# mravanelli/pytorch-kaldi

Measured on AMD Instinct MI355X. Metric: train_frames_per_sec, higher is better.
Workload: dtype bf16

## Files before the change

include/pk_amd.h:

```cpp
#ifndef PK_AMD_H
#define PK_AMD_H

#include <stdint.h>

#ifdef __cplusplus
extern "C" {
#endif

#define PK_PREC_F32 0
#define PK_PREC_BF16 1

#define PK_ACT_LINEAR 0
#define PK_ACT_RELU 1
#define PK_ACT_TANH 2
#define PK_ACT_SIGMOID 3
#define PK_ACT_LEAKY_RELU 4
#define PK_ACT_ELU 5

#define PK_CELL_LIGRU 0
#define PK_CELL_RNN 1
#define PK_CELL_LSTM 2
#define PK_CELL_GRU 3
#define PK_CELL_MINGRU 4

// ... 122 lines not shown
int pk_rec_bwd_bf16(void* stream, int cell, int act, int T, int B, int bidir, int H, const float* U, const float* mask,
                    float mask_scalar, const float* Y, const float* S, const float* dY, float* dP2, uint16_t* dGb,
                    int64_t g_pitch, int prefilled);
int pk_rec_fwd_bf16_ln(void* stream, int cell, int act, int T, int B, int bidir, int H, const float* P,
                       const float* pscale, const float* pshift, const float* U, const float* mask, float mask_scalar,
                       const float* ln_gamma, const float* ln_beta, float ln_eps, float* Y, float* S, float* LNS,
                       uint16_t* Yb, int64_t y_pitch, int prefilled, float* lnwork);
int pk_rec_bwd_bf16_ln(void* stream, int cell, int act, int T, int B, int bidir, int H, const float* U, const float* mask,
                       float mask_scalar, const float* ln_gamma, float ln_eps, const float* Y, const float* S,
                       const float* LNS, const float* dY, float* dP2, uint16_t* dGb, int64_t g_pitch, int prefilled,
                       float* lnwork, float* dln_gamma, float* dln_beta);
void pk_persist2_set_trace(void* dev_buf);
void pk_persist2_set_empty_step(int on);
void pk_persist2_set_mode(int force_safe);
void pk_persist2_set_poll_delay(int units);
void pk_persist2_set_lstm_waves(int waves);
int pk_persist2_get_lstm_waves(void);
void pk_rec_helper_set_mode(int mode);
int pk_rec_helper_get_mode(void);
int pk_rec2p_fwd_bf16(void* stream, int cell, int act, int T, int B, int bidir, int H, const float* P,
                      const float* pscale, const float* pshift, const float* U, const float* mask, float mask_scalar,
                      float* Y, float* S, uint16_t* Yb, uint16_t* Xb, int64_t y_pitch, int prefilled);
int pk_rec2p_bwd_bf16(void* stream, int cell, int act, int T, int B, int bidir, int H, const float* U, const float* mask,
                      float mask_scalar, const float* Y, const float* S, const float* dY, uint16_t* dGb, int64_t g_pitch,
                      int prefilled);
int pk_rec2p_fwd_bf16_ln(void* stream, int cell, int act, int T, int B, int bidir, int H, const float* P,
                         const float* pscale, const float* pshift, const float* U, const float* mask, float mask_scalar,
                         const float* ln_gamma, const float* ln_beta, float ln_eps, float* Y, float* S, float* LNS,
                         uint16_t* Yb, uint16_t* Xb, int64_t y_pitch, int prefilled, float* lnwork);
int pk_rec2p_bwd_bf16_ln(void* stream, int cell, int act, int T, int B, int bidir, int H, const float* U, const float* mask,
                         float mask_scalar, const float* ln_gamma, float ln_eps, const float* Y, const float* S,
                         const float* LNS, const float* dY, uint16_t* dGb, int64_t g_pitch, int prefilled, float* lnwork,
                         float* dln_gamma, float* dln_beta);
unsigned pk_persist2_error_count(void);
void pk_persist2_error_reset(void);

int pk_conv1d_pool_fwd(void* stream, const float* x, const float* w, const float* bias, int B, int Cin, int L,
                       int Cout, int K, int pool, float* y, int32_t* argmax, float* work);
int64_t pk_conv_fwd_work_floats(int Cin, int Cout, int K);
int64_t pk_conv_partial_floats(int B, int Cin, int L, int Cout, int K, int pool);
int pk_conv1d_pool_bwd(void* stream, const float* x, const float* w, const float* dy, const int32_t* argmax, int B,
                       int Cin, int L, int Cout, int K, int pool, float* dw, float* dbias, float* dx,
                       float* partial);

int pk_rmsprop_step(void* stream, float* p, const float* g, float* square_avg, int64_t n, float lr, float alpha,
                    float eps, float weight_decay);
int pk_sgd_step(void* stream, float* p, const float* g, float* momentum_buf, int64_t n, float lr, float momentum,
                float weight_decay, int first_step);
int pk_adam_step(void* stream, float* p, const float* g, float* exp_avg, float* exp_avg_sq, float* max_exp_avg_sq,
                 int64_t n, float lr, float beta1, float beta2, float eps, float weight_decay, int step);
int pk_fused_step(void* stream, int kind, float* p, float* g, float* s0, float* s1, float* s2, int64_t n, float lr, float h0,
                  float h1, float h2, float weight_decay, int step, int zero_grad, const int64_t* segs, int nseg,
                  uint16_t* shadow);

unsigned pk_persist_error_count(void);
void pk_persist_error_reset(void);

int pk_linear_bn_act_bf16_covers(int64_t M, int64_t N, int64_t K);
int pk_linear_bn_act_bf16(void* stream, int M, int N, int K, const uint16_t* xb, int64_t ldx, const uint16_t* wb, int64_t ldw,
                          const float* bias, const float* gamma, const float* beta, float eps, float momentum,
                          float* running_mean, float* running_var, int act, const float* mask, float* z, float* a,
                          float* y, uint16_t* yb, int64_t ldyb, float* mean, float* var);
int pk_gemm_bf16_small_splitk(int M, int N, int K);
int pk_linear_bn_act_bf16_sk(void* stream, int M, int N, int K, const uint16_t* xb, int64_t ldx, const uint16_t* wb,
                             int64_t ldw, const float* bias, const float* gamma, const float* beta, float eps,
                             float momentum, float* running_mean, float* running_var, int act, const float* mask,
                             float* z, float* a, float* y, uint16_t* yb, int64_t ldyb, float* mean, float* var,
                             int splitk, float* ws);
int pk_conv1d_pool_dgrad(void* stream, const float* w, const float* dy, const int32_t* argmax, int B, int Cin, int L, int Cout,
                         int K, int pool, float* dx, float* work);
int pk_conv_bf16_covers(int Cin, int Cout, int K, int pool);
int64_t pk_conv_bf16_work_floats(int B, int Cin, int L, int Cout, int K, int pool, int backward);
int pk_conv1d_pool_fwd_bf16(void* stream, const float* x, const float* w, const float* bias, int B, int Cin, int L, int Cout,
                            int K, int pool, float* y, int32_t* argmax, float* work);
int pk_conv1d_pool_bwd_bf16(void* stream, const float* x, const float* w, const float* dy, const int32_t* argmax, int B,
                            int Cin, int L, int Cout, int K, int pool, float* dw, float* dx, float* work);
int pk_selftest_mfma(void* stream, int* h_bad_count);
int pk_selftest_permlane(void* stream, int* h_bad_count);
int pk_selftest_dpp_row_sum(void* stream, int* h_bad_count);
int pk_selftest_cu_hog(void* stream, int blocks, int usec, float* buf);

typedef struct pk_ark pk_ark;
pk_ark* pk_ark_open(const char* path, int64_t offset);
void pk_ark_close(pk_ark* a);
int pk_ark_next(pk_ark* a, int key_expected, char* key, int keycap, int64_t* rows, int64_t* cols);
int pk_ark_read(pk_ark* a, float* dst);
int pk_ark_skip(pk_ark* a);
int pk_ivec_next(pk_ark* a, char* key, int keycap, int64_t* n);
int pk_ivec_read(pk_ark* a, int32_t* dst);
int pk_context_window(const float* x, int64_t rows, int64_t cols, int left, int right, float* out);
int pk_mean_var_norm(float* x, int64_t rows, int64_t cols);

#ifdef __cplusplus
}
#endif
#endif
```

pytorch-kaldi_amd/_lib.py:

```python
import ctypes
import os
import re
import threading

HERE = os.path.dirname(os.path.abspath(__file__))
LIB_PATH = os.path.join(HERE, "lib", "libpk_amd.so")
HEADER = os.path.join(HERE, "..", "include", "pk_amd.h")

_lock = threading.Lock()
_lib = None

c_void_p, c_int, c_float, c_double, c_int64 = ctypes.c_void_p, ctypes.c_int, ctypes.c_float, ctypes.c_double, ctypes.c_int64
P = c_void_p

SIGNATURES = {
    "pk_version": (c_int, []),
    "pk_last_error": (ctypes.c_char_p, []),
    "pk_num_cu": (c_int, []),
    "pk_gemm": (c_int, [P, c_int, c_int, c_int, c_int, c_float, P, c_int64, c_int64, P, c_int64, c_int64, c_float, P,
                        c_int64, P, c_int, P]),
    "pk_gemm_f32_set_form": (None, [c_int]),
    "pk_gemm_bf16_tile_m": (c_int, [c_int]),
    "pk_gemm_bf16_auto_splitk": (c_int, [c_int, c_int, c_int]),
    "pk_gemm_bf16_set_tile": (None, [c_int]),
# ... 46 lines not shown
    "pk_conv1d_pool_fwd_bf16": (c_int, [P, P, P, P, c_int, c_int, c_int, c_int, c_int, c_int, P, P, P]),
    "pk_conv1d_pool_bwd_bf16": (c_int, [P, P, P, P, P, c_int, c_int, c_int, c_int, c_int, c_int, P, P, P]),
    "pk_bn_act_bwd_small_covers": (c_int, [c_int64, c_int64]),
    "pk_bn_act_bwd_small": (c_int, [P, P, P, P, c_int, P, P, P, c_float, P, c_int64, c_int64, P, c_int64, P, P, P, P, P, P, P]),
    "pk_rec_work_floats": (c_int64, [c_int, c_int, c_int, c_int, c_int]),
    "pk_rec_ln_saved_floats": (c_int64, [c_int, c_int, c_int, c_int]),
    "pk_rec_ln_work_floats": (c_int64, [c_int, c_int, c_int, c_int]),
    "pk_rec_fwd": (c_int, [P, c_int, c_int, c_int, c_int, c_int, c_int, c_int, c_int, P, P, P, P, P, c_float, P, P, P,
                           P, P, P]),
    "pk_rec_bwd": (c_int, [P, c_int, c_int, c_int, c_int, c_int, c_int, c_int, c_int, P, P, c_float, P, P, P, P, P, P,
                           P, P, P, P]),
    "pk_rec_self_fill": (c_int, [c_int]),
    "pk_rec_plan_cus": (c_int, [c_int, c_int]),
    "pk_gemm_bf16_auto_splitk_cus": (c_int, [c_int, c_int, c_int, c_int]),
    "pk_rec_fwd_bf16": (c_int, [P, c_int, c_int, c_int, c_int, c_int, c_int, P, P, P, P, P, c_float, P, P, P, c_int64, c_int]),
    "pk_rec_bwd_bf16": (c_int, [P, c_int, c_int, c_int, c_int, c_int, c_int, P, P, c_float, P, P, P, P, P, c_int64, c_int]),
    "pk_rec2p_fwd_bf16_ln": (c_int, [P, c_int, c_int, c_int, c_int, c_int, c_int, P, P, P, P, P, c_float, P, P, c_float, P, P, P,
                                     P, P, c_int64, c_int, P]),
    "pk_rec2p_bwd_bf16_ln": (c_int, [P, c_int, c_int, c_int, c_int, c_int, c_int, P, P, c_float, P, c_float, P, P, P, P, P,
                                     c_int64, c_int, P, P, P]),
    "pk_rec_fwd_bf16_ln": (c_int, [P, c_int, c_int, c_int, c_int, c_int, c_int, P, P, P, P, P, c_float, P, P, c_float, P, P, P,
                                   P, c_int64, c_int, P]),
    "pk_rec_bwd_bf16_ln": (c_int, [P, c_int, c_int, c_int, c_int, c_int, c_int, P, P, c_float, P, c_float, P, P, P, P, P, P,
                                   c_int64, c_int, P, P, P]),
    "pk_rec2p_fwd_bf16": (c_int, [P, c_int, c_int, c_int, c_int, c_int, c_int, P, P, P, P, P, c_float, P, P, P, P, c_int64, c_int]),
    "pk_rec2p_bwd_bf16": (c_int, [P, c_int, c_int, c_int, c_int, c_int, c_int, P, P, c_float, P, P, P, P, c_int64, c_int]),
    "pk_persist2_set_trace": (None, [P]),
    "pk_persist2_set_empty_step": (None, [c_int]),
    "pk_persist2_set_mode": (None, [c_int]),
    "pk_persist2_set_poll_delay": (None, [c_int]),
    "pk_persist2_set_lstm_waves": (None, [c_int]),
    "pk_rec_helper_set_mode": (None, [c_int]),
    "pk_rec_helper_get_mode": (c_int, []),
    "pk_persist2_get_lstm_waves": (c_int, []),
    "pk_persist2_error_count": (ctypes.c_uint, []),
    "pk_persist2_error_reset": (None, []),
    "pk_conv1d_pool_fwd": (c_int, [P, P, P, P, c_int, c_int, c_int, c_int, c_int, c_int, P, P, P]),
    "pk_conv_fwd_work_floats": (c_int64, [c_int, c_int, c_int]),
    "pk_conv_partial_floats": (c_int64, [c_int, c_int, c_int, c_int, c_int, c_int]),
    "pk_conv1d_pool_bwd": (c_int, [P, P, P, P, P, c_int, c_int, c_int, c_int, c_int, c_int, P, P, P, P]),
    "pk_ark_open": (P, [ctypes.c_char_p, c_int64]),
    "pk_ark_close": (None, [P]),
    "pk_ark_next": (c_int, [P, c_int, ctypes.c_char_p, c_int, ctypes.POINTER(c_int64), ctypes.POINTER(c_int64)]),
    "pk_ark_read": (c_int, [P, P]),
    "pk_ark_skip": (c_int, [P]),
    "pk_ivec_next": (c_int, [P, ctypes.c_char_p, c_int, ctypes.POINTER(c_int64)]),
    "pk_ivec_read": (c_int, [P, P]),
    "pk_context_window": (c_int, [P, c_int64, c_int64, c_int, c_int, P]),
    "pk_mean_var_norm": (c_int, [P, c_int64, c_int64]),
    "pk_rmsprop_step": (c_int, [P, P, P, P, c_int64, c_float, c_float, c_float, c_float]),
    "pk_sgd_step": (c_int, [P, P, P, P, c_int64, c_float, c_float, c_float, c_int]),
    "pk_adam_step": (c_int, [P, P, P, P, P, P, c_int64, c_float, c_float, c_float, c_float, c_float, c_int]),
    "pk_fused_step": (c_int, [P, c_int, P, P, P, P, P, c_int64, c_float, c_float, c_float, c_float, c_float, c_int, c_int, P, c_int, P]),
    "pk_persist_error_count": (ctypes.c_uint, []),
    "pk_persist_error_reset": (None, []),
    "pk_linear_bn_act_bf16_covers": (c_int, [c_int64, c_int64, c_int64]),
    "pk_linear_bn_act_bf16": (c_int, [P, c_int, c_int, c_int, P, c_int64, P, c_int64, P, P, P, c_float, c_float, P, P, c_int, P,
                                      P, P, P, P, c_int64, P, P]),
    "pk_gemm_bf16_small_splitk": (c_int, [c_int, c_int, c_int]),
    "pk_linear_bn_act_bf16_sk": (c_int, [P, c_int, c_int, c_int, P, c_int64, P, c_int64, P, P, P, c_float, c_float, P, P, c_int, P,
                                         P, P, P, P, c_int64, P, P, c_int, P]),
    "pk_selftest_mfma": (c_int, [P, ctypes.POINTER(c_int)]),
    "pk_selftest_permlane": (c_int, [P, ctypes.POINTER(c_int)]),
    "pk_selftest_dpp_row_sum": (c_int, [P, ctypes.POINTER(c_int)]),
    "pk_selftest_cu_hog": (c_int, [P, c_int, c_int, P]),
}


def declared_symbols():
    with open(HEADER) as f:
        text = re.sub(r"/\*.*?\*/", "", f.read(), flags=re.S)
    return sorted(set(re.findall(r"\b(pk_[a-z0-9_]+)\s*\(", text)))


class PkError(RuntimeError):
    pass


def _map_torch_hip_runtime():
    import torch

    hip = os.path.join(os.path.dirname(torch.__file__), "lib", "libamdhip64.so")
    if os.path.exists(hip):
        ctypes.CDLL(hip, mode=ctypes.RTLD_GLOBAL)
    return hip


def hip_runtimes_mapped():
    try:
        with open("/proc/self/maps") as f:
            return {line.split()[-1] for line in f if "libamdhip64" in line}
    except OSError:
        return set()


def load():
    global _lib
    if _lib is not None:
        return _lib
    with _lock:
        if _lib is not None:
            return _lib
        if not os.path.exists(LIB_PATH):
            raise PkError(
                "libpk_amd.so is not built (%s). Run `python -c 'import __graft_entry__ as g; g.build()'`; "
                "this engine has no CPU fallback." % LIB_PATH)
# ... 169 lines not shown
```

pytorch-kaldi_amd/csrc/pk_optim.hip:

```cpp
#include "pk_common.h"

namespace {

__global__ void rmsprop_kernel(float* __restrict__ p, const float* __restrict__ g, float* __restrict__ sq, long n, float lr,
                               float alpha, float eps, float wd) {
    for (long i = blockIdx.x * (long)blockDim.x + threadIdx.x; i < n; i += (long)gridDim.x * blockDim.x) {
        float gv = g[i];
        const float pv = p[i];
        if (wd != 0.f) gv += wd * pv;
        const float s = alpha * sq[i] + (1.f - alpha) * gv * gv;
        sq[i] = s;
        p[i] = pv - lr * gv / (sqrtf(s) + eps);
    }
}

__global__ void sgd_kernel(float* __restrict__ p, const float* __restrict__ g, float* __restrict__ buf, long n, float lr,
                           float momentum, float wd, int first) {
    for (long i = blockIdx.x * (long)blockDim.x + threadIdx.x; i < n; i += (long)gridDim.x * blockDim.x) {
        float gv = g[i];
        const float pv = p[i];
        if (wd != 0.f) gv += wd * pv;
        if (momentum != 0.f) {
            const float b = first ? gv : momentum * buf[i] + gv;
            buf[i] = b;
            gv = b;
        }
        p[i] = pv - lr * gv;
    }
}

__global__ void adam_kernel(float* __restrict__ p, const float* __restrict__ g, float* __restrict__ m, float* __restrict__ v,
                            float* __restrict__ vmax, long n, float lr, float beta1, float beta2, float eps, float wd,
                            float bc1, float bc2s) {
    for (long i = blockIdx.x * (long)blockDim.x + threadIdx.x; i < n; i += (long)gridDim.x * blockDim.x) {
        float gv = g[i];
        const float pv = p[i];
        if (wd != 0.f) gv += wd * pv;
        const float mv = beta1 * m[i] + (1.f - beta1) * gv;
        float vv = beta2 * v[i] + (1.f - beta2) * gv * gv;
        m[i] = mv;
        v[i] = vv;
        if (vmax != nullptr) {
            vv = fmaxf(vmax[i], vv);
            vmax[i] = vv;
        }
        const float denom = sqrtf(vv) / bc2s + eps;
        p[i] = pv - (lr / bc1) * (mv / denom);
    }
}

template <int KIND>
__global__ void fused_step_kernel(float* __restrict__ p, float* __restrict__ g, float* __restrict__ s0, float* __restrict__ s1,
                                  float* __restrict__ s2, long n, float lr, float h0, float h1, float h2, float wd, float bc1,
                                  float bc2s, int first, int zero_grad, const long* __restrict__ segs, int nseg,
                                  unsigned short* __restrict__ shadow) {
    for (long i = 4 * (blockIdx.x * (long)blockDim.x + threadIdx.x); i < n; i += 4 * (long)gridDim.x * blockDim.x) {
        f32x4 gv = *reinterpret_cast<const f32x4*>(g + i);
        f32x4 pv = *reinterpret_cast<const f32x4*>(p + i);
        if (wd != 0.f) {
#pragma unroll
            for (int e = 0; e < 4; ++e) gv[e] += wd * pv[e];
        }
        if (KIND == 0) {
            f32x4 sq = *reinterpret_cast<const f32x4*>(s0 + i);
#pragma unroll
            for (int e = 0; e < 4; ++e) {
                sq[e] = h0 * sq[e] + (1.f - h0) * gv[e] * gv[e];
                pv[e] = pv[e] - lr * gv[e] / (sqrtf(sq[e]) + h1);
            }
            *reinterpret_cast<f32x4*>(s0 + i) = sq;
        } else if (KIND == 1) {
            if (h0 != 0.f) {
                f32x4 b = *reinterpret_cast<const f32x4*>(s0 + i);
#pragma unroll
                for (int e = 0; e < 4; ++e) {
                    b[e] = first ? gv[e] : h0 * b[e] + gv[e];
                    gv[e] = b[e];
                }
                *reinterpret_cast<f32x4*>(s0 + i) = b;
            }
#pragma unroll
            for (int e = 0; e < 4; ++e) pv[e] = pv[e] - lr * gv[e];
        } else {
            f32x4 m = *reinterpret_cast<const f32x4*>(s0 + i), v = *reinterpret_cast<const f32x4*>(s1 + i);
            f32x4 vm = v;
#pragma unroll
            for (int e = 0; e < 4; ++e) {
                m[e] = h0 * m[e] + (1.f - h0) * gv[e];
                v[e] = h1 * v[e] + (1.f - h1) * gv[e] * gv[e];
                vm[e] = v[e];
            }
            *reinterpret_cast<f32x4*>(s0 + i) = m;
            *reinterpret_cast<f32x4*>(s1 + i) = v;
            if (s2 != nullptr) {
                const f32x4 old = *reinterpret_cast<const f32x4*>(s2 + i);
#pragma unroll
                for (int e = 0; e < 4; ++e) vm[e] = fmaxf(old[e], v[e]);
                *reinterpret_cast<f32x4*>(s2 + i) = vm;
            }
#pragma unroll
            for (int e = 0; e < 4; ++e) pv[e] = pv[e] - (lr / bc1) * (m[e] / (sqrtf(vm[e]) / bc2s + h2));
        }
        *reinterpret_cast<f32x4*>(p + i) = pv;
        if (zero_grad) *reinterpret_cast<f32x4*>(g + i) = f32x4{0.f, 0.f, 0.f, 0.f};
        if (nseg > 0) {
            int lo = 0, hi = nseg;
            while (hi - lo > 1) {
                const int mid = (lo + hi) >> 1;
                if (segs[5 * mid] <= i) lo = mid;
                else hi = mid;
            }
            const long off = segs[5 * lo], rows = segs[5 * lo + 1], cols = segs[5 * lo + 2], pitch = segs[5 * lo + 3], soff = segs[5 * lo + 4];
            const long rel = i - off;
            if (rel >= 0 && rel < rows * cols) {
                const long row = rel / cols, col = rel - row * cols;
                uint2 pk;
                pk.x = pk_pack_bf2(pv[0], pv[1]);
                pk.y = pk_pack_bf2(pv[2], pv[3]);
                *reinterpret_cast<uint2*>(shadow + soff + row * pitch + col) = pk;
            }
        }
    }
}

inline int blocks_for(long n) {
    long b = (n + 255) / 256;
    if (b > 4096) b = 4096;
    if (b < 1) b = 1;
    return (int)b;
}

}

extern "C" int pk_rmsprop_step(void* stream, float* p, const float* g, float* square_avg, int64_t n, float lr, float alpha,
                               float eps, float weight_decay) {
    if (n == 0) return 0;
    hipLaunchKernelGGL(rmsprop_kernel, dim3(blocks_for(n)), dim3(256), 0, pk_stream(stream), p, g, square_avg, (long)n, lr,
                       alpha, eps, weight_decay);
    PK_LAUNCH_CHECK();
    return 0;
}

extern "C" int pk_sgd_step(void* stream, float* p, const float* g, float* momentum_buf, int64_t n, float lr,
                           float momentum, float weight_decay, int first_step) {
    if (n == 0) return 0;
    PK_REQUIRE(momentum == 0.f || momentum_buf != nullptr, "pk_sgd_step: momentum needs a buffer");
    hipLaunchKernelGGL(sgd_kernel, dim3(blocks_for(n)), dim3(256), 0, pk_stream(stream), p, g, momentum_buf, (long)n, lr,
                       momentum, weight_decay, first_step);
    PK_LAUNCH_CHECK();
    return 0;
}

extern "C" int pk_adam_step(void* stream, float* p, const float* g, float* exp_avg, float* exp_avg_sq, float* max_exp_avg_sq,
                            int64_t n, float lr, float beta1, float beta2, float eps, float weight_decay, int step) {
    if (n == 0) return 0;
    PK_REQUIRE(step >= 1 && exp_avg != nullptr && exp_avg_sq != nullptr, "pk_adam_step: step counts from 1 and needs both moments");
    const float bc1 = 1.f - powf(beta1, (float)step);
    const float bc2s = sqrtf(1.f - powf(beta2, (float)step));
    hipLaunchKernelGGL(adam_kernel, dim3(blocks_for(n)), dim3(256), 0, pk_stream(stream), p, g, exp_avg, exp_avg_sq,
                       max_exp_avg_sq, (long)n, lr, beta1, beta2, eps, weight_decay, bc1, bc2s);
    PK_LAUNCH_CHECK();
    return 0;
}

extern "C" int pk_fused_step(void* stream, int kind, float* p, float* g, float* s0, float* s1, float* s2, int64_t n, float lr,
                             float h0, float h1, float h2, float weight_decay, int step, int zero_grad, const int64_t* segs,
                             int nseg, uint16_t* shadow) {
    if (n == 0) return 0;
    PK_REQUIRE(kind >= 0 && kind <= 2 && step >= 1, "pk_fused_step: kind 0..2, step counts from 1");
    PK_REQUIRE((n & 3) == 0 && (((uintptr_t)p | (uintptr_t)g | (uintptr_t)s0 | (uintptr_t)s1 | (uintptr_t)s2) & 15) == 0,
               "pk_fused_step: n and the buffers must be multiples of 4 elements / 16-byte aligned");
    PK_REQUIRE(kind != 0 || s0 != nullptr, "pk_fused_step: RMSprop needs its square average");
    PK_REQUIRE(kind != 1 || h0 == 0.f || s0 != nullptr, "pk_fused_step: momentum needs a buffer");
    PK_REQUIRE(kind != 2 || (s0 != nullptr && s1 != nullptr), "pk_fused_step: Adam needs both moments");
    PK_REQUIRE(nseg == 0 || (segs != nullptr && shadow != nullptr && ((uintptr_t)shadow & 7) == 0), "pk_fused_step: null segment table / copy");
    const float bc1 = kind == 2 ? 1.f - powf(h0, (float)step) : 1.f;
    const float bc2s = kind == 2 ? sqrtf(1.f - powf(h1, (float)step)) : 1.f;
    const dim3 grid(blocks_for(n / 4)), block(256);
    hipStream_t st = pk_stream(stream);
    const long* sg = reinterpret_cast<const long*>(segs);
    if (kind == 0) hipLaunchKernelGGL(fused_step_kernel<0>, grid, block, 0, st, p, g, s0, s1, s2, (long)n, lr, h0, h1, h2, weight_decay, bc1, bc2s, 0, zero_grad, sg, nseg, (unsigned short*)shadow);
    else if (kind == 1) hipLaunchKernelGGL(fused_step_kernel<1>, grid, block, 0, st, p, g, s0, s1, s2, (long)n, lr, h0, h1, h2, weight_decay, bc1, bc2s, step == 1 ? 1 : 0, zero_grad, sg, nseg, (unsigned short*)shadow);
    else hipLaunchKernelGGL(fused_step_kernel<2>, grid, block, 0, st, p, g, s0, s1, s2, (long)n, lr, h0, h1, h2, weight_decay, bc1, bc2s, 0, zero_grad, sg, nseg, (unsigned short*)shadow);
    PK_LAUNCH_CHECK();
    return 0;
}
```

pytorch-kaldi_amd/functional.py:

```python
import ctypes
import os
import weakref

import torch

from . import _lib

PREC = {"fp32": 0, "bf16": 1}
ACT = {"linear": 0, "relu": 1, "tanh": 2, "sigmoid": 3, "leaky_relu": 4, "elu": 5}
CELL = {"liGRU": 0, "RNN": 1, "LSTM": 2, "GRU": 3, "minimalGRU": 4}
REC_STEPWISE, REC_PERSISTENT = 0, 1


class _Settings:

    def __init__(self):
        self.precision = os.environ.get("PK_PRECISION", "fp32")
        self.rec_algo = os.environ.get("PK_REC_ALGO", "auto")
        self.mask_rng = os.environ.get("PK_MASK_RNG", "device")
        assert self.mask_rng in ("reference", "reference_host", "device"), self.mask_rng
        self.wgrad_side = _lib.experiment("wgrad_side", "1") != "0"
        self.self_fill = _lib.experiment("rec_self_fill", "1") != "0"
        self.side_late = _lib.experiment("side_late", "1") != "0"
        self.side_cus = _lib.experiment("side_cus", "0") != "0"
# ... 233 lines not shown


def _rows2d(x):
    if x.dim() != 2:
        x = x.reshape(-1, x.shape[-1])
    if x.stride(1) != 1 or (x.shape[0] > 1 and x.stride(0) < x.shape[1]):
        x = x.contiguous()
    return x


def _new(*shape, like):
    return torch.empty(*shape, device=like.device, dtype=torch.float32)


def _splitk(out_tiles, K):
    if K < 4096:
        return 1
    slots = int(_lib.experiment("f32_splitk_slots", "1024"))
    s = max(1, slots // max(1, out_tiles))
    return int(min(16, s, max(1, K // 1024)))


def _small_m_splitk(M, N, K):
    if M > 256 or K < 512 or _lib.experiment("f32_small_splitk", "1") == "0":
        return 1
    return int(max(1, min(16, 512 // max(1, _tiles(M, N)), K // 64)))


def gemm(M, N, K, A, a_rs, a_cs, B, b_rs, b_cs, C, ldc, alpha=1.0, beta=0.0, bias=None, splitk=1, prec=None):
    lib = _lib.load()
    ws = None
    if splitk == 1 and a_cs == 1 and (prec or settings.precision) == "fp32":
        splitk = _small_m_splitk(M, N, K)
    if splitk > 1:
        ws = torch.empty(splitk * M * N, device=C.device, dtype=torch.float32)
    rc = lib.pk_gemm(_stream(), PREC[prec or settings.precision], M, N, K, alpha, _p(A), a_rs, a_cs, _p(B), b_rs, b_cs,
                     beta, _p(C), ldc, _p(bias), splitk, _p(ws))
    _lib.check(rc, "pk_gemm")
    return C


def _tiles(M, N):
    return ((M + 127) // 128) * ((N + 127) // 128)


def _tiles_bf(M, N):
    return (M, N)


def _up(n, m):
    return (n + m - 1) // m * m


def weight_bf16(w):
    sh = getattr(w, "_pk_shadow", None)
    if sh is not None:
        view, version, alive, flat_version = sh
        if alive() is not None:
            owner = getattr(w, "_pk_owner", None)
            owner = owner() if owner is not None else None
            fv = owner.flat._version if owner is not None else flat_version
            if w._version == version and fv == flat_version:
                return view
            cvt_bf16(w.detach(), out=view)
            w._pk_shadow = (view, w._version, alive, fv)
            return view
    owner = getattr(w, "_pk_owner", None)
    owner = owner() if owner is not None else None
    if owner is not None and w.is_contiguous():
        owner.want_shadow(w)
    return cvt_bf16(w.contiguous())


def cvt_bf16(x2, nseg=1, seglen=None, segpad=None, out=None):
    lib = _lib.load()
    rows, cols = x2.shape
    if seglen is None:
        nseg, seglen = 1, cols
    if segpad is None:
        segpad = _up(seglen, 8)
    assert nseg * seglen == cols and x2.stride(1) == 1
    pitch = _up(nseg * segpad, 64)
    if out is None:
        out = torch.empty(rows, pitch, device=x2.device, dtype=torch.bfloat16)
    assert tuple(out.shape) == (rows, pitch) and out.dtype == torch.bfloat16 and out.is_contiguous()
    _lib.check(lib.pk_cvt_bf16(_stream(), _p(x2), x2.stride(0), rows, nseg, seglen, segpad, _p(out), pitch),
               "pk_cvt_bf16")
    return out


_SMALL_SPLITK = _lib.experiment("small_splitk", "1") != "0"


def gemm_bf16(M, N, K, A, lda, a_kc, B, ldb, b_kc, C, ldc, alpha=1.0, beta=0.0, bias=None, splitk=1):
    lib = _lib.load()
    ws = None
    if splitk == 1 and a_kc and M <= 128 and _SMALL_SPLITK:
        splitk = int(lib.pk_gemm_bf16_small_splitk(M, N, K))
    if splitk > 1:
        ws = torch.empty(splitk * M * N, device=C.device, dtype=torch.float32)

    def ptr(t):
        if isinstance(t, tuple):
            return ctypes.c_void_p(t[0].data_ptr() + 2 * t[1])
        return ctypes.c_void_p(t.data_ptr())

    rc = lib.pk_gemm_bf16(_stream(), M, N, K, alpha, ptr(A), lda, int(a_kc), ptr(B), ldb, int(b_kc), beta, _p(C), ldc,
                          _p(bias), splitk, _p(ws))
    _lib.check(rc, "pk_gemm_bf16")
    return C


def gemm_bf16_bn_stats(M, N, K, A, lda, a_kc, B, ldb, b_kc, C, ldc, bias=None, gates=None):
    lib = _lib.load()

    def done(mean, var):
        return (mean, var) if gates is None else (mean, var) + tuple(bn_finalize_gates(mean, var, *gates))

    if _lib.experiment("gemm_stats", "1") == "0":
        gemm_bf16(M, N, K, A, lda, a_kc, B, ldb, b_kc, C, ldc, bias=bias)
        return done(*bn_stats(C if ldc == N else C.as_strided((M, N), (ldc, 1))))
    stats = torch.empty(int(lib.pk_gemm_bf16_stats_floats(M, N)), device=C.device, dtype=torch.float32)
    rb = ctypes.c_int(0)
    rc = lib.pk_gemm_bf16_stats(_stream(), M, N, K, 1.0, _p(A), lda, int(a_kc), _p(B), ldb, int(b_kc), _p(C), ldc, _p(bias),
# ... 1265 lines not shown
    if cell not in ("liGRU", "RNN", "LSTM", "GRU", "minimalGRU") or H > 576 or use_ln:
        return False
    return training or not use_bn or not torch.is_grad_enabled()


class _Prefill:
    stream = None

    def __init__(self):
        self.done = 0

    def start(self, *bufs):
        if not settings.wgrad_side:
            return
        main = torch.cuda.current_stream()
        if _Prefill.stream is None:
            _Prefill.stream = torch.cuda.Stream()
        st = _Prefill.stream
        st.wait_stream(main)
        with torch.cuda.stream(st):
            for b in bufs:
                if b is not None:
                    b.view(torch.int16).fill_(-1)
        for b in bufs:
            if b is not None:
                b.record_stream(st)
        self.done = 1

    def wait(self):
        if self.done:
            torch.cuda.current_stream().wait_stream(_Prefill.stream)


class RecLayerPerfFn(torch.autograd.Function):

    @staticmethod
    def forward(ctx, x, xb_in, Wcat, bcat, Ucat, gamma, beta, running_mean, running_var, mask, cfg, edge=None):
        ctx.set_materialize_grads(False)
        _need_gpu(x, Wcat, bcat, Ucat, gamma, beta, mask)
        lib = _lib.load()
        cell, act, H, bidir, use_bn, training, eps, momentum, mask_scalar, xseg = cfg[:10]
        ctx.wparams, ctx.uparams = (cfg[10], cfg[11]) if len(cfg) > 10 else (None, None)
        ctx.side_w, ctx.side_u = (bool(cfg[12]), bool(cfg[13])) if len(cfg) > 13 else (False, False)
        ctx.affine = cfg[15] if len(cfg) > 15 else None
        T, B, D = x.shape
        G = lib.pk_rec_num_gates(CELL[cell])
        NS = lib.pk_rec_num_saved(CELL[cell])
        ndir = 2 if bidir else 1
        TB, GH = T * B, G * H
        Wcat = Wcat.contiguous()
        Ucat = Ucat.contiguous()
        if xb_in is None:
            xseg = None
            xb, Wb, K = cvt_bf16(_rows2d(x)), cvt_bf16(Wcat), D
        else:
            nseg, seglen, segpad = xseg
            assert nseg * seglen == D and xb_in.shape[0] == TB
            xb, Wb, K = xb_in, cvt_bf16(Wcat, nseg, seglen, segpad), nseg * segpad
            assert Wb.shape[1] == xb.shape[1]
        Hp = _up(H, 8)
        Yb = torch.empty(TB, _up(ndir * Hp, 64), device=x.device, dtype=torch.bfloat16)
        two_phase = cell in ("GRU", "minimalGRU")
        self_fill = settings.self_fill and lib.pk_rec_self_fill(CELL[cell]) == 1
        dGb = None
        if any(ctx.needs_input_grad) and not self_fill:
            dGb = torch.empty(ndir * TB, _up(G * Hp, 64), device=x.device, dtype=torch.bfloat16)
        Xb = torch.empty_like(Yb) if two_phase else None
        fill = _Prefill()
        if not self_fill:
            fill.start(Yb, Xb, dGb)
        P = _new(TB, GH, like=Wcat)
        mean = var = None
        bn_bufs = cfg[14] if len(cfg) > 14 else None
        pscale = pshift = None
        if use_bn and training and bn_bufs is not None:
            mean, var, pscale, pshift = gemm_bf16_bn_stats(TB, GH, K, xb, xb.shape[1], 1, Wb, Wb.shape[1], 1, P, GH, gates=(
                gamma, beta, eps, H, bn_bufs[0], bn_bufs[1], bn_bufs[2], momentum, ndir * TB))
        elif use_bn and training:
            mean, var = gemm_bf16_bn_stats(TB, GH, K, xb, xb.shape[1], 1, Wb, Wb.shape[1], 1, P, GH)
        else:
            gemm_bf16(TB, GH, K, xb, xb.shape[1], 1, Wb, Wb.shape[1], 1, P, GH)
        if use_bn:
            if pscale is not None:
                pass
            elif training:
                pscale, pshift = bn_finalize(mean, var, gamma, beta, eps, running_mean, running_var, momentum, ndir * TB)
            else:
                mean, var = running_mean, running_var
                pscale, pshift = bn_finalize(mean, var, gamma, beta, eps)
        else:
            pscale = torch.ones(GH, device=x.device)
            pshift = bcat.contiguous() if bcat is not None else torch.zeros(GH, device=x.device)
        infer = not any(ctx.needs_input_grad) and _Kinks.queue is None and _lib.experiment("fwd_nosave", "1") != "0"
        keep_y = bool(cfg[16]) if len(cfg) > 16 else True
        Y = _new(T, B, ndir * H, like=Wcat)
        S = None if infer else _new(ndir, TB, NS * H, like=Wcat)
        Yarg = Y if (keep_y or not infer) else None
        _lib.raise_if_persist_failed()
        fill.wait()
        if two_phase:
            rc = lib.pk_rec2p_fwd_bf16(_stream(), CELL[cell], ACT[act], T, B, int(bidir), H, _p(P), _p(pscale),
                                       _p(pshift), _p(Ucat), _p(mask), float(mask_scalar), _p(Yarg), _p(S), _p(Yb), _p(Xb),
                                       Yb.shape[1], 2 if self_fill else fill.done)
            _lib.check(rc, "pk_rec2p_fwd_bf16")
        else:
            rc = lib.pk_rec_fwd_bf16(_stream(), CELL[cell], ACT[act], T, B, int(bidir), H, _p(P), _p(pscale), _p(pshift),
                                     _p(Ucat), _p(mask), float(mask_scalar), _p(Yarg), _p(S), _p(Yb), Yb.shape[1],
                                     2 if self_fill else fill.done)
            _lib.check(rc, "pk_rec_fwd_bf16")
        if S is not None:
            _force_kinks(S, cell, T, B, ndir, H)
# ... 56 lines not shown
        elif not side_u:
            do_dU()
        dPb = torch.empty(TB, _up(GH, 64), device=dY.device, dtype=torch.bfloat16)
        part = _new(int(lib.pk_bn_partial_floats(TB, GH)), like=dY)
        sum_g = _new(GH, like=dY)
        sum_gx = _new(GH, like=dY) if use_bn else None
        g1 = ctypes.c_void_p(dGb.data_ptr() + 2 * TB * Gp) if bidir else None
        acc_g = acc_b = None
        if use_bn and ctx.affine is not None:
            acc_g = adjacent_view([q.grad for q in ctx.affine[0]])
            acc_b = adjacent_view([q.grad for q in ctx.affine[1]])
            if acc_g is None or acc_b is None:
                raise _lib.PkError("perf-mode recurrent layer: the BatchNorm gradients left the flat buffer between forward "
                                   "and backward (optim.FlatParams.zero_grad() re-aliases them)")
        rc = lib.pk_bn_bwd_bf16(_stream(), _p(dGb), g1, Gp, G, H, _p(P), GH, TB, _p(mean) if use_bn else None,
                                _p(var) if use_bn else None, eps, _p(gamma) if use_bn else None, float(TB), _p(part),
                                _p(sum_g), _p(sum_gx), _p(dPb), dPb.shape[1], _p(acc_b), _p(acc_g))
        _lib.check(rc, "pk_bn_bwd_bf16")
        dgamma = dbeta = dbias = None
        if use_bn and acc_g is None:
            dgamma, dbeta = sum_gx, sum_g
        elif not use_bn and ctx.has_bias:
            dbias = sum_g
        Kx = D if xseg is None else xseg[0] * xseg[2]
        dWp = _new(GH, Kx, like=dY)
        dW = None

        def do_dW():
            nonlocal dW
            gview = adjacent_view([q.grad for q in ctx.wparams]) if side_w else None
            sk = _splitk_bf(_tiles_bf(GH, Kx), TB)
            if gview is not None and xseg is None:
                gemm_bf16(GH, Kx, TB, dPb, dPb.shape[1], 0, xb, xb.shape[1], 0, gview, Kx, beta=1.0, splitk=sk)
                return
            gemm_bf16(GH, Kx, TB, dPb, dPb.shape[1], 0, xb, xb.shape[1], 0, dWp, Kx, splitk=sk)
            if gview is not None:
                nseg, seglen, segpad = xseg
                with torch.no_grad():
                    for s_ in range(nseg):
                        gview[:, s_ * seglen:(s_ + 1) * seglen].add_(dWp[:, s_ * segpad:s_ * segpad + seglen])
                return
            if xseg is None:
                dW = dWp
            else:
                nseg, seglen, segpad = xseg
                dW = torch.cat([dWp[:, s_ * segpad:s_ * segpad + seglen] for s_ in range(nseg)], 1)
            if side_w:
                _accumulate_rows(ctx.wparams, [dW[g * H:(g + 1) * H] for g in range(G)])

        if side_w and not late:
            side_launch(do_dW, (dPb, xb, dWp), ctx.wparams)
        dx = None
        if ctx.needs_input_grad[0]:
            Wb2 = Wb if xseg is None else cvt_bf16(Wcat)
            dx = _new(TB, D, like=dY)
            gemm_bf16(TB, D, GH, dPb, dPb.shape[1], 1, Wb2, Wb2.shape[1], 0, dx, D)
            dx = dx.view(T, B, D)
        if late:
            free = 0
            if settings.side_cus:
                held = int(lib.pk_rec_plan_cus(ndir * B, H))
                free = max(int(lib.pk_num_cu()) - held, 0) if held > 0 else 0
            if side_u:
                side_launch(_sized_for(free, do_dU), (Y, S, Yb, dGb, Xb, dU), ctx.uparams)
            if side_w:
                side_launch(_sized_for(free, do_dW), (dPb, xb, dWp), ctx.wparams)
        if not side_w:
            do_dW()
        return dx, None, (None if side_w else dW), dbias, (None if side_u else dU), dgamma, dbeta, None, None, None, None, None


CONV_BF16_DEFAULT = "1"


def conv_bf16_mode():
    return os.environ.get("PK_CONV_BF16", CONV_BF16_DEFAULT)


class ConvPoolFn(torch.autograd.Function):
    @staticmethod
    def forward(ctx, x, w, bias, pool):
        _need_gpu(x, w, bias)
        lib = _lib.load()
        x = x.contiguous()
        w = w.contiguous()
        B, Cin, L = x.shape
        Cout, _, K = w.shape
        Lp = (L - K + 1) // pool
        y = _new(B, Cout, Lp, like=x)
        arg = torch.empty(B, Cout, Lp, device=x.device, dtype=torch.int32)
        mode = conv_bf16_mode()
        ctx.conv_bf = (bf16_mode() and mode in ("1", "2") and (Cin >= 8 or mode == "2")
                       and lib.pk_conv_bf16_covers(Cin, Cout, K, pool) == 1)
        if ctx.conv_bf:
            work = _new(int(lib.pk_conv_bf16_work_floats(B, Cin, L, Cout, K, pool, 0)), like=x)
            _lib.check(lib.pk_conv1d_pool_fwd_bf16(_stream(), _p(x), _p(w), _p(bias), B, Cin, L, Cout, K, pool, _p(y),
                                                   ctypes.c_void_p(arg.data_ptr()), _p(work)), "pk_conv1d_pool_fwd_bf16")
        else:
            work = _new(int(lib.pk_conv_fwd_work_floats(Cin, Cout, K)), like=x)
            _lib.check(lib.pk_conv1d_pool_fwd(_stream(), _p(x), _p(w), _p(bias), B, Cin, L, Cout, K, pool, _p(y),
                                              ctypes.c_void_p(arg.data_ptr()), _p(work)), "pk_conv1d_pool_fwd")
        if _Decisions.pool is not None:
            fpool, off = _Decisions.pool.pop(0)
            assert fpool == pool and tuple(off.shape) == (B, Cout, Lp), (fpool, pool, tuple(off.shape), (B, Cout, Lp))
            forced = (torch.arange(Lp, device=x.device, dtype=torch.int32) * pool)[None, None, :] + off.to(x.device).to(torch.int32)
            _Decisions.report.append(("pool", int((forced != arg).sum()), arg.numel()))
            arg = forced.contiguous()
# ... 38 lines not shown
```

pytorch-kaldi_amd/optim.py:

```python
import ctypes
import os
import weakref

import torch

from . import _lib


def _stream():
    return ctypes.c_void_p(torch.cuda.current_stream().cuda_stream)


class FlatParams:
    def __init__(self, module, align=64):
        self.module = module
        self.params = [p for p in module.parameters()]
        dev = self.params[0].device
        unused = {id(p) for p in module.pk_unused_parameters()} if hasattr(module, "pk_unused_parameters") else set()
        self.unused = [id(p) in unused for p in self.params]
        index = {id(p): i for i, p in enumerate(self.params)}
        units, placed = [], set()
        if hasattr(module, "pk_flat_groups") and _lib.experiment("flat_groups", "1") != "0":
            for grp in module.pk_flat_groups():
                ids = [index[id(q)] for q in grp if id(q) in index and id(q) not in unused and index[id(q)] not in placed]
                if ids:
                    units.append(ids)
                    placed.update(ids)
        for i in range(len(self.params)):
            if not self.unused[i] and i not in placed:
                units.append([i])
        self.offsets = [0] * len(self.params)
        off = 0
        for ids in units:
            off = (off + align - 1) // align * align
            for i in ids:
                self.offsets[i] = off
                off += self.params[i].numel()
        off = (off + align - 1) // align * align
        self.n_active = off
        for i, p in enumerate(self.params):
            if self.unused[i]:
                self.offsets[i] = off
                off += (p.numel() + align - 1) // align * align
        self.numel = off
        self.flat = torch.zeros(off, device=dev, dtype=torch.float32)
        self.grad = torch.zeros(off, device=dev, dtype=torch.float32)
        with torch.no_grad():
            for p, o in zip(self.params, self.offsets):
                n = p.numel()
                self.flat[o:o + n].copy_(p.detach().reshape(-1))
                p.data = self.flat[o:o + n].view(p.shape)
                p.grad = self.grad[o:o + n].view(p.shape)
                p._pk_flat = True
                p._pk_owner = weakref.ref(self)
        self._index = {id(p): i for i, p in enumerate(self.params)}
        self._clean = False
        self._shadow_req = set()
        self._shadow_have = ()
        self.shadow = self.shadow_segs = None

    def want_shadow(self, p):
        i = self._index.get(id(p))
        if (i is not None and not self.unused[i] and p.dim() == 2 and p.shape[1] % 4 == 0 and self.offsets[i] % 4 == 0
                and p.is_cuda):
            self._shadow_req.add(i)

    def invalidate_shadows(self):
        for p in self.params:
            sh = getattr(p, "_pk_shadow", None)
            if sh is not None:
                p._pk_shadow = (sh[0], -1, sh[2], -1)

    def build_shadows(self):
        from . import functional as F_
        want = tuple(sorted(self._shadow_req, key=lambda i: self.offsets[i]))
        if want == self._shadow_have:
            return
        rows = []
        soff = 0
        for i in want:
            p = self.params[i]
            pitch = (p.shape[1] + 63) // 64 * 64
            rows.append((self.offsets[i], p.shape[0], p.shape[1], pitch, soff))
            soff += p.shape[0] * pitch
        self.shadow = torch.zeros(max(soff, 8), device=self.flat.device, dtype=torch.bfloat16)
        self.shadow_segs = torch.tensor(rows, dtype=torch.int64, device=self.flat.device).reshape(-1, 5)
        self._shadow_have = want
        for i, (_o, r, c, pitch, so) in zip(want, rows):
            p = self.params[i]
            view = self.shadow[so:so + r * pitch].view(r, pitch)
            F_.cvt_bf16(p.detach(), out=view)
            p._pk_shadow = (view, p._version, weakref.ref(self.shadow), self.flat._version)

    def zero_grad(self):
        from .functional import join_side
        join_side()
        if self._clean:
            self._clean = False
        else:
            self.grad.zero_()
        for p, o in zip(self.params, self.offsets):
            if p.grad is None or p.grad.data_ptr() != self.grad.data_ptr() + 4 * o:
                p.grad = self.grad[o:o + p.numel()].view(p.shape)


def _flat_mark_dirty(self):
    self._clean = False


FlatParams.mark_dirty = _flat_mark_dirty


class FusedOptimizer:

    _STATE_KEYS = {"rmsprop": ("square_avg",), "sgd": ("momentum_buffer",),
                   "adam": ("exp_avg", "exp_avg_sq", "max_exp_avg_sq")}

    def __init__(self, flat, kind, lr, alpha=0.99, eps=1e-8, momentum=0.0, weight_decay=0.0, centered=False,
                 dampening=0.0, nesterov=False, betas=(0.9, 0.999), amsgrad=False):
        if kind not in ("rmsprop", "sgd", "adam"):
            raise _lib.PkError("fused optimizer covers rmsprop, sgd and adam (got %s)" % kind)
        if kind == "rmsprop" and (momentum != 0.0 or centered):
            raise _lib.PkError("fused RMSprop is the momentum-free, non-centred form every shipped recipe uses")
        if kind == "sgd" and (dampening != 0.0 or nesterov):
            raise _lib.PkError("fused SGD does not implement dampening / nesterov")
        self.flat, self.kind, self.lr = flat, kind, lr
        self.alpha, self.eps, self.momentum, self.weight_decay = alpha, eps, momentum, weight_decay
        self.betas, self.amsgrad = tuple(betas), bool(amsgrad)
        z = lambda: torch.zeros_like(flat.flat)
        self.bufs = {}
        if kind == "rmsprop":
            self.bufs["square_avg"] = z()
        elif kind == "sgd" and momentum != 0.0:
            self.bufs["momentum_buffer"] = z()
        elif kind == "adam":
            self.bufs["exp_avg"], self.bufs["exp_avg_sq"] = z(), z()
            if self.amsgrad:
                self.bufs["max_exp_avg_sq"] = z()
        self.steps = 0
        self.param_groups = [{"lr": lr}]
        self.zero_in_step = False

    @property
    def state(self):
        return next(iter(self.bufs.values()), None)

    def zero_grad(self):
        self.flat.zero_grad()

    def step(self):
        if not self.flat.flat.is_cuda:
            raise _lib.PkError("fused optimizer step runs on the GPU only (no CPU fallback)")
        from .functional import join_side
        join_side()
        lib = _lib.load()
        lr = float(self.param_groups[0]["lr"])
        f = self.flat
        ptr = lambda k: self.bufs[k].data_ptr() if k in self.bufs else None
        if f.n_active % 4 == 0 and _lib.experiment("fused_step", "1") != "0":
            if f._shadow_req and not torch.cuda.is_current_stream_capturing():
                f.build_shadows()
            nseg = len(f._shadow_have)
            zero = bool(self.zero_in_step) and _lib.experiment("opt_zero_in_step", "1") != "0"
            kind = {"rmsprop": 0, "sgd": 1, "adam": 2}[self.kind]
            h = {"rmsprop": (self.alpha, self.eps, 0.0), "sgd": (self.momentum, 0.0, 0.0),
                 "adam": (self.betas[0], self.betas[1], self.eps)}[self.kind]
            s0 = ptr("square_avg") if kind == 0 else ptr("momentum_buffer") if kind == 1 else ptr("exp_avg")
            rc = lib.pk_fused_step(_stream(), kind, f.flat.data_ptr(), f.grad.data_ptr(), s0, ptr("exp_avg_sq"),
                                   ptr("max_exp_avg_sq"), f.n_active, lr, h[0], h[1], h[2], self.weight_decay, self.steps + 1,
                                   int(zero), f.shadow_segs.data_ptr() if nseg else None, nseg,
                                   f.shadow.data_ptr() if nseg else None)
            _lib.check(rc, "fused optimizer step")
            f._clean = zero
            self.steps += 1
            return
        if self.kind == "rmsprop":
            rc = lib.pk_rmsprop_step(_stream(), f.flat.data_ptr(), f.grad.data_ptr(), ptr("square_avg"), f.n_active, lr,
                                     self.alpha, self.eps, self.weight_decay)
        elif self.kind == "sgd":
            rc = lib.pk_sgd_step(_stream(), f.flat.data_ptr(), f.grad.data_ptr(), ptr("momentum_buffer"), f.n_active, lr,
                                 self.momentum, self.weight_decay, int(self.steps == 0))
        else:
            rc = lib.pk_adam_step(_stream(), f.flat.data_ptr(), f.grad.data_ptr(), ptr("exp_avg"), ptr("exp_avg_sq"),
                                  ptr("max_exp_avg_sq"), f.n_active, lr, self.betas[0], self.betas[1], self.eps,
                                  self.weight_decay, self.steps + 1)
        _lib.check(rc, "fused optimizer step")
        self.steps += 1

    def _torch_twin(self):
        import torch.optim as optim
        ps = self.flat.params
        lr = float(self.param_groups[0]["lr"])
        if self.kind == "rmsprop":
            return optim.RMSprop(ps, lr=lr, alpha=self.alpha, eps=self.eps, weight_decay=self.weight_decay)
        if self.kind == "sgd":
            return optim.SGD(ps, lr=lr, momentum=self.momentum, weight_decay=self.weight_decay)
        return optim.Adam(ps, lr=lr, betas=self.betas, eps=self.eps, weight_decay=self.weight_decay, amsgrad=self.amsgrad)

    def state_dict(self):
        sd = self._torch_twin().state_dict()
        state = {}
        if self.steps > 0:
            for i, (p, o) in enumerate(zip(self.flat.params, self.flat.offsets)):
                if self.flat.unused[i]:
                    continue
                ent = {k: b[o:o + p.numel()].view(p.shape).clone() for k, b in self.bufs.items()}
                if self.kind != "sgd":
                    ent["step"] = torch.tensor(float(self.steps))
                if ent:
                    state[i] = ent
        sd["state"] = state
        return sd

    def load_state_dict(self, sd):
        groups = sd["param_groups"]
        if len(groups) != 1 or len(groups[0]["params"]) != len(self.flat.params):
            raise _lib.PkError("optimizer state does not match this architecture's parameter list")
        g = groups[0]
        self.param_groups[0]["lr"] = g["lr"]
        self.weight_decay = float(g.get("weight_decay", self.weight_decay))
        if self.kind == "rmsprop":
# ... 48 lines not shown
```

Measured before the change: 3.816 million.

## Cache bf16 shadows of concatenated recurrent weights, refreshed inside fused optimizer step

Extends the optimizer's bf16 shadow mechanism to concatenated recurrent weight matrices, including segmented or padded layouts. The fused step kernel now writes these bf16 copies directly, using an 8-wide segment descriptor that carries segment length and padding. The recurrent layer forward and backward passes then reuse the cached copy instead of converting the fp32 weight to bf16 on every call. This adds a multi-segment lookup with scattered stores to the optimizer kernel, and shadow rebuilds now depend on a simple size signature, which could miss changes in the request set.

```diff
diff --git a/include/pk_amd.h b/include/pk_amd.h
--- a/include/pk_amd.h
+++ b/include/pk_amd.h
@@ -198,6 +198,9 @@
 int pk_fused_step(void* stream, int kind, float* p, float* g, float* s0, float* s1, float* s2, int64_t n, float lr, float h0,
                   float h1, float h2, float weight_decay, int step, int zero_grad, const int64_t* segs, int nseg,
                   uint16_t* shadow);
+int pk_fused_step_seg(void* stream, int kind, float* p, float* g, float* s0, float* s1, float* s2, int64_t n, float lr,
+                      float h0, float h1, float h2, float weight_decay, int step, int zero_grad, const int64_t* segs,
+                      int nseg, uint16_t* shadow);
 
 unsigned pk_persist_error_count(void);
 void pk_persist_error_reset(void);
diff --git a/pytorch-kaldi_amd/_lib.py b/pytorch-kaldi_amd/_lib.py
--- a/pytorch-kaldi_amd/_lib.py
+++ b/pytorch-kaldi_amd/_lib.py
@@ -122,6 +122,7 @@
     "pk_sgd_step": (c_int, [P, P, P, P, c_int64, c_float, c_float, c_float, c_int]),
     "pk_adam_step": (c_int, [P, P, P, P, P, P, c_int64, c_float, c_float, c_float, c_float, c_float, c_int]),
     "pk_fused_step": (c_int, [P, c_int, P, P, P, P, P, c_int64, c_float, c_float, c_float, c_float, c_float, c_int, c_int, P, c_int, P]),
+    "pk_fused_step_seg": (c_int, [P, c_int, P, P, P, P, P, c_int64, c_float, c_float, c_float, c_float, c_float, c_int, c_int, P, c_int, P]),
     "pk_persist_error_count": (ctypes.c_uint, []),
     "pk_persist_error_reset": (None, []),
     "pk_linear_bn_act_bf16_covers": (c_int, [c_int64, c_int64, c_int64]),
diff --git a/pytorch-kaldi_amd/csrc/pk_optim.hip b/pytorch-kaldi_amd/csrc/pk_optim.hip
--- a/pytorch-kaldi_amd/csrc/pk_optim.hip
+++ b/pytorch-kaldi_amd/csrc/pk_optim.hip
@@ -53,7 +53,7 @@
 __global__ void fused_step_kernel(float* __restrict__ p, float* __restrict__ g, float* __restrict__ s0, float* __restrict__ s1,
                                   float* __restrict__ s2, long n, float lr, float h0, float h1, float h2, float wd, float bc1,
                                   float bc2s, int first, int zero_grad, const long* __restrict__ segs, int nseg,
-                                  unsigned short* __restrict__ shadow) {
+                                  int segw, unsigned short* __restrict__ shadow) {
     for (long i = 4 * (blockIdx.x * (long)blockDim.x + threadIdx.x); i < n; i += 4 * (long)gridDim.x * blockDim.x) {
         f32x4 gv = *reinterpret_cast<const f32x4*>(g + i);
         f32x4 pv = *reinterpret_cast<const f32x4*>(p + i);
@@ -107,17 +107,28 @@
             int lo = 0, hi = nseg;
             while (hi - lo > 1) {
                 const int mid = (lo + hi) >> 1;
-                if (segs[5 * mid] <= i) lo = mid;
+                if (segs[segw * mid] <= i) lo = mid;
                 else hi = mid;
             }
-            const long off = segs[5 * lo], rows = segs[5 * lo + 1], cols = segs[5 * lo + 2], pitch = segs[5 * lo + 3], soff = segs[5 * lo + 4];
-            const long rel = i - off;
-            if (rel >= 0 && rel < rows * cols) {
+            const long off = segs[segw * lo];
+            for (; lo >= 0 && segs[segw * lo] == off; --lo) {
+                const long* sg = segs + segw * lo;
+                const long rows = sg[1], cols = sg[2], pitch = sg[3], soff = sg[4];
+                const long rel = i - off;
+                if (rel < 0 || rel >= rows * cols) continue;
                 const long row = rel / cols, col = rel - row * cols;
-                uint2 pk;
-                pk.x = pk_pack_bf2(pv[0], pv[1]);
-                pk.y = pk_pack_bf2(pv[2], pv[3]);
-                *reinterpret_cast<uint2*>(shadow + soff + row * pitch + col) = pk;
+                const long seglen = segw > 5 ? sg[5] : cols, segpad = segw > 5 ? sg[6] : cols;
+                unsigned short* dst = shadow + soff + row * pitch;
+                if (seglen == cols) {
+                    uint2 pk;
+                    pk.x = pk_pack_bf2(pv[0], pv[1]);
+                    pk.y = pk_pack_bf2(pv[2], pv[3]);
+                    *reinterpret_cast<uint2*>(dst + col) = pk;
+                } else {
+                    const long c1 = col + 2, s0i = col / seglen, s1i = c1 / seglen;
+                    *reinterpret_cast<unsigned*>(dst + s0i * segpad + (col - s0i * seglen)) = pk_pack_bf2(pv[0], pv[1]);
+                    *reinterpret_cast<unsigned*>(dst + s1i * segpad + (c1 - s1i * seglen)) = pk_pack_bf2(pv[2], pv[3]);
+                }
             }
         }
     }
@@ -163,9 +174,9 @@
     return 0;
 }
 
-extern "C" int pk_fused_step(void* stream, int kind, float* p, float* g, float* s0, float* s1, float* s2, int64_t n, float lr,
-                             float h0, float h1, float h2, float weight_decay, int step, int zero_grad, const int64_t* segs,
-                             int nseg, uint16_t* shadow) {
+static int fused_step_impl(void* stream, int kind, float* p, float* g, float* s0, float* s1, float* s2, int64_t n, float lr,
+                           float h0, float h1, float h2, float weight_decay, int step, int zero_grad, const int64_t* segs,
+                           int nseg, int segw, uint16_t* shadow) {
     if (n == 0) return 0;
     PK_REQUIRE(kind >= 0 && kind <= 2 && step >= 1, "pk_fused_step: kind 0..2, step counts from 1");
     PK_REQUIRE((n & 3) == 0 && (((uintptr_t)p | (uintptr_t)g | (uintptr_t)s0 | (uintptr_t)s1 | (uintptr_t)s2) & 15) == 0,
@@ -179,9 +190,21 @@
     const dim3 grid(blocks_for(n / 4)), block(256);
     hipStream_t st = pk_stream(stream);
     const long* sg = reinterpret_cast<const long*>(segs);
-    if (kind == 0) hipLaunchKernelGGL(fused_step_kernel<0>, grid, block, 0, st, p, g, s0, s1, s2, (long)n, lr, h0, h1, h2, weight_decay, bc1, bc2s, 0, zero_grad, sg, nseg, (unsigned short*)shadow);
-    else if (kind == 1) hipLaunchKernelGGL(fused_step_kernel<1>, grid, block, 0, st, p, g, s0, s1, s2, (long)n, lr, h0, h1, h2, weight_decay, bc1, bc2s, step == 1 ? 1 : 0, zero_grad, sg, nseg, (unsigned short*)shadow);
-    else hipLaunchKernelGGL(fused_step_kernel<2>, grid, block, 0, st, p, g, s0, s1, s2, (long)n, lr, h0, h1, h2, weight_decay, bc1, bc2s, 0, zero_grad, sg, nseg, (unsigned short*)shadow);
-    PK_LAUNCH_CHECK();
-    return 0;
-}
+    if (kind == 0) hipLaunchKernelGGL(fused_step_kernel<0>, grid, block, 0, st, p, g, s0, s1, s2, (long)n, lr, h0, h1, h2, weight_decay, bc1, bc2s, 0, zero_grad, sg, nseg, segw, (unsigned short*)shadow);
+    else if (kind == 1) hipLaunchKernelGGL(fused_step_kernel<1>, grid, block, 0, st, p, g, s0, s1, s2, (long)n, lr, h0, h1, h2, weight_decay, bc1, bc2s, step == 1 ? 1 : 0, zero_grad, sg, nseg, segw, (unsigned short*)shadow);
+    else hipLaunchKernelGGL(fused_step_kernel<2>, grid, block, 0, st, p, g, s0, s1, s2, (long)n, lr, h0, h1, h2, weight_decay, bc1, bc2s, 0, zero_grad, sg, nseg, segw, (unsigned short*)shadow);
+    PK_LAUNCH_CHECK();
+    return 0;
+}
+
+extern "C" int pk_fused_step(void* stream, int kind, float* p, float* g, float* s0, float* s1, float* s2, int64_t n, float lr,
+                             float h0, float h1, float h2, float weight_decay, int step, int zero_grad, const int64_t* segs,
+                             int nseg, uint16_t* shadow) {
+    return fused_step_impl(stream, kind, p, g, s0, s1, s2, n, lr, h0, h1, h2, weight_decay, step, zero_grad, segs, nseg, 5, shadow);
+}
+
+extern "C" int pk_fused_step_seg(void* stream, int kind, float* p, float* g, float* s0, float* s1, float* s2, int64_t n, float lr,
+                                 float h0, float h1, float h2, float weight_decay, int step, int zero_grad, const int64_t* segs,
+                                 int nseg, uint16_t* shadow) {
+    return fused_step_impl(stream, kind, p, g, s0, s1, s2, n, lr, h0, h1, h2, weight_decay, step, zero_grad, segs, nseg, 8, shadow);
+}
diff --git a/pytorch-kaldi_amd/functional.py b/pytorch-kaldi_amd/functional.py
--- a/pytorch-kaldi_amd/functional.py
+++ b/pytorch-kaldi_amd/functional.py
@@ -309,7 +309,9 @@
     return (n + m - 1) // m * m
 
 
-def weight_bf16(w):
+def weight_bf16(w, nseg=1, seglen=None, segpad=None, params=None):
+    if params is not None or seglen is not None:
+        return _cat_weight_bf16(w, nseg, seglen, segpad, params)
     sh = getattr(w, "_pk_shadow", None)
     if sh is not None:
         view, version, alive, flat_version = sh
@@ -327,6 +329,31 @@
     if owner is not None and w.is_contiguous():
         owner.want_shadow(w)
     return cvt_bf16(w.contiguous())
+
+
+def _cat_weight_bf16(w, nseg, seglen, segpad, params):
+    if seglen is None:
+        nseg, seglen = 1, w.shape[1]
+    if segpad is None:
+        segpad = _up(seglen, 8)
+    owner = getattr(params[0], "_pk_owner", None) if params else None
+    owner = owner() if owner is not None else None
+    key = None
+    if owner is not None and _lib.experiment("rec_weight_copies", "1") != "0":
+        key = owner.cat_key(w, params, nseg, seglen, segpad)
+    if key is None:
+        return cvt_bf16(w.contiguous(), nseg, seglen, segpad)
+    sh = owner._cat_shadow.get(key)
+    if sh is not None and sh[2]() is not None:
+        view, versions, alive, flat_version = sh
+        now = tuple(q._version for q in params)
+        if versions == now and flat_version == owner.flat._version:
+            return view
+        cvt_bf16(w, nseg, seglen, segpad, out=view)
+        owner._cat_shadow[key] = (view, now, alive, owner.flat._version)
+        return view
+    owner.want_cat_shadow(key, params)
+    return cvt_bf16(w, nseg, seglen, segpad)
 
 
 def cvt_bf16(x2, nseg=1, seglen=None, segpad=None, out=None):
@@ -1698,11 +1725,11 @@
         Ucat = Ucat.contiguous()
         if xb_in is None:
             xseg = None
-            xb, Wb, K = cvt_bf16(_rows2d(x)), cvt_bf16(Wcat), D
+            xb, Wb, K = cvt_bf16(_rows2d(x)), weight_bf16(Wcat, params=ctx.wparams), D
         else:
             nseg, seglen, segpad = xseg
             assert nseg * seglen == D and xb_in.shape[0] == TB
-            xb, Wb, K = xb_in, cvt_bf16(Wcat, nseg, seglen, segpad), nseg * segpad
+            xb, Wb, K = xb_in, weight_bf16(Wcat, nseg, seglen, segpad, params=ctx.wparams), nseg * segpad
             assert Wb.shape[1] == xb.shape[1]
         Hp = _up(H, 8)
         Yb = torch.empty(TB, _up(ndir * Hp, 64), device=x.device, dtype=torch.bfloat16)
@@ -1865,7 +1892,7 @@
             side_launch(do_dW, (dPb, xb, dWp), ctx.wparams)
         dx = None
         if ctx.needs_input_grad[0]:
-            Wb2 = Wb if xseg is None else cvt_bf16(Wcat)
+            Wb2 = Wb if xseg is None else weight_bf16(Wcat, params=ctx.wparams)
             dx = _new(TB, D, like=dY)
             gemm_bf16(TB, D, GH, dPb, dPb.shape[1], 1, Wb2, Wb2.shape[1], 0, dx, D)
             dx = dx.view(T, B, D)
diff --git a/pytorch-kaldi_amd/optim.py b/pytorch-kaldi_amd/optim.py
--- a/pytorch-kaldi_amd/optim.py
+++ b/pytorch-kaldi_amd/optim.py
@@ -57,6 +57,8 @@
         self._clean = False
         self._shadow_req = set()
         self._shadow_have = ()
+        self._cat_req = {}
+        self._cat_shadow = {}
         self.shadow = self.shadow_segs = None
 
     def want_shadow(self, p):
@@ -65,32 +67,69 @@
                 and p.is_cuda):
             self._shadow_req.add(i)
 
+    def cat_key(self, w, params, nseg, seglen, segpad):
+        i = self._index.get(id(params[0])) if params else None
+        if i is None or w.dim() != 2 or not w.is_cuda or not w.is_contiguous() or w.dtype != torch.float32:
+            return None
+        off, (rows, cols) = self.offsets[i], w.shape
+        if (w.data_ptr() != self.flat.data_ptr() + 4 * off or off + rows * cols > self.n_active
+                or sum(q.numel() for q in params) != rows * cols or any(self._index.get(id(q)) is None for q in params)):
+            return None
+        if cols % 4 or off % 4 or nseg * seglen != cols or seglen % 2 or segpad % 2 or segpad < seglen:
+            return None
+        return (off, rows, cols, nseg, seglen, segpad)
+
+    def want_cat_shadow(self, key, params):
+        self._cat_req.setdefault(key, tuple(params))
+
     def invalidate_shadows(self):
         for p in self.params:
             sh = getattr(p, "_pk_shadow", None)
             if sh is not None:
                 p._pk_shadow = (sh[0], -1, sh[2], -1)
+        for k, sh in self._cat_shadow.items():
+            self._cat_shadow[k] = (sh[0], None, sh[2], -1)
 
     def build_shadows(self):
         from . import functional as F_
+        sig = (len(self._shadow_req), len(self._cat_req))
+        if sig == getattr(self, "_shadow_sig", None):
+            return
+        self._shadow_sig = sig
         want = tuple(sorted(self._shadow_req, key=lambda i: self.offsets[i]))
-        if want == self._shadow_have:
+        ents = [((self.offsets[i],) + tuple(self.params[i].shape) + (1, self.params[i].shape[1], self.params[i].shape[1]), i)
+                for i in want] + [(k, None) for k in self._cat_req]
+        ents.sort(key=lambda e: (e[0][:3], e[1] is None, e[0][3:]))
+        kept, last = [], None
+        for key, i in ents:
+            rng = key[:3]
+            if last is not None and rng != last and key[0] < last[0] + last[1] * last[2]:
+                continue
+            kept.append((key, i))
+            last = rng
+        have = tuple(k for k, _ in kept)
+        if have == self._shadow_have:
             return
         rows = []
         soff = 0
-        for i in want:
-            p = self.params[i]
-            pitch = (p.shape[1] + 63) // 64 * 64
-            rows.append((self.offsets[i], p.shape[0], p.shape[1], pitch, soff))
-            soff += p.shape[0] * pitch
+        for (off, r, c, nseg, seglen, segpad), i in kept:
+            pitch = (nseg * segpad + 63) // 64 * 64 if i is None else (c + 63) // 64 * 64
+            rows.append((off, r, c, pitch, soff, seglen, segpad, 0))
+            soff += r * pitch
         self.shadow = torch.zeros(max(soff, 8), device=self.flat.device, dtype=torch.bfloat16)
-        self.shadow_segs = torch.tensor(rows, dtype=torch.int64, device=self.flat.device).reshape(-1, 5)
-        self._shadow_have = want
-        for i, (_o, r, c, pitch, so) in zip(want, rows):
-            p = self.params[i]
+        self.shadow_segs = torch.tensor(rows, dtype=torch.int64, device=self.flat.device).reshape(-1, 8)
+        self._shadow_have = have
+        self._cat_shadow = {}
+        for (key, i), (off, r, c, pitch, so, seglen, segpad, _z) in zip(kept, rows):
             view = self.shadow[so:so + r * pitch].view(r, pitch)
-            F_.cvt_bf16(p.detach(), out=view)
-            p._pk_shadow = (view, p._version, weakref.ref(self.shadow), self.flat._version)
+            if i is not None:
+                p = self.params[i]
+                F_.cvt_bf16(p.detach(), out=view)
+                p._pk_shadow = (view, p._version, weakref.ref(self.shadow), self.flat._version)
+            else:
+                ps = self._cat_req[key]
+                F_.cvt_bf16(self.flat[off:off + r * c].view(r, c), key[3], seglen, segpad, out=view)
+                self._cat_shadow[key] = (view, tuple(q._version for q in ps), weakref.ref(self.shadow), self.flat._version)
 
     def zero_grad(self):
         from .functional import join_side
@@ -158,7 +197,7 @@
         f = self.flat
         ptr = lambda k: self.bufs[k].data_ptr() if k in self.bufs else None
         if f.n_active % 4 == 0 and _lib.experiment("fused_step", "1") != "0":
-            if f._shadow_req and not torch.cuda.is_current_stream_capturing():
+            if (f._shadow_req or f._cat_req) and not torch.cuda.is_current_stream_capturing():
                 f.build_shadows()
             nseg = len(f._shadow_have)
             zero = bool(self.zero_in_step) and _lib.experiment("opt_zero_in_step", "1") != "0"
@@ -166,7 +205,7 @@
             h = {"rmsprop": (self.alpha, self.eps, 0.0), "sgd": (self.momentum, 0.0, 0.0),
                  "adam": (self.betas[0], self.betas[1], self.eps)}[self.kind]
             s0 = ptr("square_avg") if kind == 0 else ptr("momentum_buffer") if kind == 1 else ptr("exp_avg")
-            rc = lib.pk_fused_step(_stream(), kind, f.flat.data_ptr(), f.grad.data_ptr(), s0, ptr("exp_avg_sq"),
+            rc = lib.pk_fused_step_seg(_stream(), kind, f.flat.data_ptr(), f.grad.data_ptr(), s0, ptr("exp_avg_sq"),
                                    ptr("max_exp_avg_sq"), f.n_active, lr, h[0], h[1], h[2], self.weight_decay, self.steps + 1,
                                    int(zero), f.shadow_segs.data_ptr() if nseg else None, nseg,
                                    f.shadow.data_ptr() if nseg else None)
```

After: 3.837 million (median of 2 runs). About the same (+0.5%).
